# TUMFTM/CamRaDepth

Hardware: AMD Instinct MI355X
Metric: training images/sec at 256x416 bf16 (higher is better)
Workload: dtype bf16; 1 GPU; CamRaDepth base (image+radar) train step, 8x7x256x416 per GPU, bf16 MFMA / fp32 accumulate, diffGradNorm + OneCycleLR, Dropout2d/DropPath on; global_batch=8, parallelism=dp1, hip_graph=True

## Files before the change

camradepth_amd/csrc/decoder_ops.hip:

```cpp
#include "common.h"

namespace {

constexpr int TPB = 256;
__device__ __constant__ float WO[4] = {-0.10546875f, 0.87890625f, 0.26171875f, -0.03515625f};
__device__ __constant__ float WE[4] = {-0.03515625f, 0.26171875f, 0.87890625f, -0.10546875f};

__device__ __forceinline__ void taps_of(int o, int n, int (&idx)[4], float (&w)[4]) {
  const int k = o >> 1;
  const bool odd = o & 1;
  const int base = odd ? k - 1 : k - 2;
#pragma unroll
  for (int t = 0; t < 4; ++t) {
    int i = base + t;
    idx[t] = i < 0 ? 0 : (i > n - 1 ? n - 1 : i);
    w[t] = odd ? WO[t] : WE[t];
  }
}

template <int F8>
__global__ __launch_bounds__(TPB) void k_bicubic(const bf16_t* x, int x_ld, int H, int W, int C, void* y, int y_ld, float inv_scale,
                                                 void* y2, int y2_ld) {
  const int b = blockIdx.y;
  const int CG = C >> 3;
  const int OW = 2 * W;
  const long long total = (long long)H * W * CG;
  const long long i = (long long)blockIdx.x * TPB + threadIdx.x;
  if (i >= total) return;
  const int cg = (int)(i % CG);
  const int pix = (int)(i / CG);
  const int k = pix / W, m = pix - k * W;
  const bf16_t* xb = x + (long long)b * H * W * x_ld + cg * 8;
  int cx[5];
#pragma unroll
  for (int c = 0; c < 5; ++c) { const int ix = m - 2 + c; cx[c] = ix < 0 ? 0 : (ix > W - 1 ? W - 1 : ix); }
  float he[5][8], ho[5][8];
#pragma unroll
  for (int r = 0; r < 5; ++r) {
    int iy = k - 2 + r;
    iy = iy < 0 ? 0 : (iy > H - 1 ? H - 1 : iy);
    float v[5][8];
#pragma unroll
    for (int c = 0; c < 5; ++c) load8(xb, ((long long)iy * W + cx[c]) * x_ld, 0, v[c]);
#pragma unroll
    for (int j = 0; j < 8; ++j) { he[r][j] = 0.f; ho[r][j] = 0.f; }
#pragma unroll
    for (int t = 0; t < 4; ++t)
#pragma unroll
      for (int j = 0; j < 8; ++j) { he[r][j] += WE[t] * v[t][j]; ho[r][j] += WO[t] * v[t + 1][j]; }
  }
#pragma unroll
  for (int oy = 0; oy < 2; ++oy)
#pragma unroll
    for (int ox = 0; ox < 2; ++ox) {
      float out[8];
#pragma unroll
      for (int j = 0; j < 8; ++j) out[j] = 0.f;
#pragma unroll
      for (int t = 0; t < 4; ++t) {
        const float wy = oy ? WO[t] : WE[t];
#pragma unroll
        for (int j = 0; j < 8; ++j) out[j] += wy * (ox ? ho[t + oy][j] : he[t + oy][j]);
      }
      const long long opix = (long long)b * 2 * H * OW + (long long)(2 * k + oy) * OW + 2 * m + ox;
      if (F8) store8_fp8(y, opix * y_ld + cg * 8, out, inv_scale);
      else store8_bf16(y, opix * y_ld + cg * 8, out);
      if (F8 == 2) store8_bf16(y2, opix * y2_ld + cg * 8, out);
    }
}

__device__ __forceinline__ void bwd_weights(int i, int n, float (&w)[10]) {
#pragma unroll
  for (int k = 0; k < 10; ++k) {
    const int o = 2 * i - 4 + k;
    float acc = 0.f;
    if (o >= 0 && o < 2 * n) {
      int idx[4];
      float ww[4];
      taps_of(o, n, idx, ww);
#pragma unroll
      for (int t = 0; t < 4; ++t)
        if (idx[t] == i) acc += ww[t];
    }
    w[k] = acc;
  }
}

__global__ __launch_bounds__(TPB) void k_bicubic_bwd(const bf16_t* dy, int dy_ld, int H, int W, int C, bf16_t* dx, int dx_ld,
                                                     int accumulate) {
  const int b = blockIdx.y;
  const int CG = C >> 3;
  const int OH = 2 * H, OW = 2 * W;
  const long long total = (long long)H * W * CG;
  const long long i = (long long)blockIdx.x * TPB + threadIdx.x;
  if (i >= total) return;
  const int cg = (int)(i % CG);
  const int pix = (int)(i / CG);
  const int iy = pix / W, ix = pix - iy * W;
  float wy[10], wx[10];
  bwd_weights(iy, H, wy);
  bwd_weights(ix, W, wx);
  const bf16_t* db = dy + (long long)b * OH * OW * dy_ld + cg * 8;
  float out[8];
#pragma unroll
  for (int j = 0; j < 8; ++j) out[j] = 0.f;
  const bool border = iy < 2 || iy > H - 3 || ix < 2 || ix > W - 3;
  if (!border) {
#pragma unroll
    for (int a = 1; a < 9; ++a) {
      const int oy = 2 * iy - 4 + a;
#pragma unroll
      for (int c = 1; c < 9; ++c) {
        const int ox = 2 * ix - 4 + c;
        float v[8];
        load8(db, ((long long)oy * OW + ox) * dy_ld, 0, v);
        const float w = wy[a] * wx[c];
#pragma unroll
        for (int j = 0; j < 8; ++j) out[j] += w * v[j];
      }
    }
  } else {
    for (int a = 0; a < 10; ++a) {
      const int oy = 2 * iy - 4 + a;
      if (oy < 0 || oy >= OH || wy[a] == 0.f) continue;
      for (int c = 0; c < 10; ++c) {
        const int ox = 2 * ix - 4 + c;
        if (ox < 0 || ox >= OW || wx[c] == 0.f) continue;
        float v[8];
        load8(db, ((long long)oy * OW + ox) * dy_ld, 0, v);
        const float w = wy[a] * wx[c];
#pragma unroll
        for (int j = 0; j < 8; ++j) out[j] += w * v[j];
      }
    }
  }
  const long long off = ((long long)b * H * W + pix) * dx_ld + cg * 8;
  if (accumulate) {
    float o[8];
    load8(dx, off, 0, o);
#pragma unroll
    for (int j = 0; j < 8; ++j) out[j] += o[j];
  }
  store8_bf16(dx, off, out);
}

__global__ __launch_bounds__(TPB) void k_nchw_to_pm(const float* x, int C, long long HW, bf16_t* y, int y_ld, int Cpad) {
  const int b = blockIdx.y;
  const int CG = Cpad >> 3;
  const long long total = HW * CG;
  for (long long i = (long long)blockIdx.x * TPB + threadIdx.x; i < total; i += (long long)gridDim.x * TPB) {
    const long long p = i % HW;
    const int cg = (int)(i / HW);
    float v[8];
#pragma unroll
    for (int j = 0; j < 8; ++j) {
      const int c = cg * 8 + j;
      v[j] = c < C ? x[((long long)b * C + c) * HW + p] : 0.f;
    }
    store8_bf16(y, ((long long)b * HW + p) * y_ld + cg * 8, v);
  }
}

__global__ __launch_bounds__(TPB) void k_pm_to_nchw(const void* x, int x_f32, int x_ld, int C, long long HW, float* y) {
  const int b = blockIdx.y;
  const long long total = HW * C;
  for (long long i = (long long)blockIdx.x * TPB + threadIdx.x; i < total; i += (long long)gridDim.x * TPB) {
    const long long p = i % HW;
    const int c = (int)(i / HW);
    const long long off = ((long long)b * HW + p) * x_ld + c;
    y[((long long)b * C + c) * HW + p] = x_f32 ? reinterpret_cast<const float*>(x)[off] : bf2f(reinterpret_cast<const bf16_t*>(x)[off]);
  }
}

__global__ __launch_bounds__(TPB) void k_scale_f32(const float* src, float* dst, long long n, float scale) {
  for (long long i = (long long)blockIdx.x * TPB + threadIdx.x; i < n; i += (long long)gridDim.x * TPB) dst[i] = scale * src[i];
}

__global__ __launch_bounds__(TPB) void k_seg_argmax(const float* logits, int ld, long long rows, int C, int num_classes,
                                                    void* y, int y_f32, int y_ld) {
  for (long long r = (long long)blockIdx.x * TPB + threadIdx.x; r < rows; r += (long long)gridDim.x * TPB) {
    const float* p = logits + r * ld;
    float best = p[0];
    int bi = 0;
    for (int c = 1; c < C; ++c) {
      float v = p[c];
      if (v > best) { best = v; bi = c; }
    }
    const float v = (float)bi / (float)num_classes;
    if (y_f32) reinterpret_cast<float*>(y)[r * y_ld] = v;
    else reinterpret_cast<bf16_t*>(y)[r * y_ld] = f2bf(v);
  }
}

__global__ __launch_bounds__(TPB) void k_slice_copy(const bf16_t* src, int s_ld, bf16_t* dst, int d_ld, long long rows, int C,
                                                    int accumulate) {
  const int CG = C >> 3;
  const long long total = rows * CG;
  for (long long i = (long long)blockIdx.x * TPB + threadIdx.x; i < total; i += (long long)gridDim.x * TPB) {
    const int cg = (int)(i % CG);
    const long long r = i / CG;
    uint4 u = *reinterpret_cast<const uint4*>(src + r * s_ld + cg * 8);
    if (accumulate) {
      float a[8], o[8];
      load8(src, r * s_ld + cg * 8, 0, a);
      load8(dst, r * d_ld + cg * 8, 0, o);
#pragma unroll
      for (int j = 0; j < 8; ++j) a[j] += o[j];
      store8_bf16(dst, r * d_ld + cg * 8, a);
    } else {
      *reinterpret_cast<uint4*>(dst + r * d_ld + cg * 8) = u;
    }
  }
}

__global__ __launch_bounds__(TPB) void k_f32_to_bf16_rows(const float* src, int s_ld, bf16_t* dst, int d_ld, long long rows,
                                                          int C, const float* scale, long long rows_per_sample,
                                                          const bf16_t* add, int add_ld, int vec) {
  if (vec) {
    const int CG = C >> 3;
    const long long total = rows * CG;
    for (long long i = (long long)blockIdx.x * TPB + threadIdx.x; i < total; i += (long long)gridDim.x * TPB) {
      const int cg = (int)(i % CG);
      const long long r = i / CG;
      const float s = scale ? scale[r / rows_per_sample] : 1.f;
      float v[8];
      load8(src, r * s_ld + cg * 8, 1, v);
#pragma unroll
      for (int j = 0; j < 8; ++j) v[j] *= s;
      if (add) {
        float a[8];
        load8(add, r * add_ld + cg * 8, 0, a);
#pragma unroll
        for (int j = 0; j < 8; ++j) v[j] += a[j];
      }
      store8_bf16(dst, r * d_ld + cg * 8, v);
    }
    return;
  }
  const long long total = rows * C;
  for (long long i = (long long)blockIdx.x * TPB + threadIdx.x; i < total; i += (long long)gridDim.x * TPB) {
    const int c = (int)(i % C);
    const long long r = i / C;
    float s = scale ? scale[r / rows_per_sample] : 1.f;
    float v = s * src[r * s_ld + c];
    if (add) v += bf2f(add[r * add_ld + c]);
    dst[r * d_ld + c] = f2bf(v);
  }
}

__global__ __launch_bounds__(TPB) void k_sigmoid_bwd(const bf16_t* a, bf16_t* da, long long n8) {
  for (long long i = (long long)blockIdx.x * TPB + threadIdx.x; i < n8; i += (long long)gridDim.x * TPB) {
    float av[8], dv[8];
    load8(a, i * 8, 0, av);
    load8(da, i * 8, 0, dv);
#pragma unroll
    for (int j = 0; j < 8; ++j) dv[j] *= av[j] * (1.f - av[j]);
    store8_bf16(da, i * 8, dv);
  }
}

__global__ __launch_bounds__(TPB) void k_head2_fwd(const bf16_t* a, const float* w, const float* bias, int H, int W,
                                                   float* depth, bf16_t* copy, int copy_ld) {
  const int b = blockIdx.y, q = threadIdx.x & 3;
  float wv[9][8];
#pragma unroll
  for (int t = 0; t < 9; ++t)
#pragma unroll
    for (int j = 0; j < 8; ++j) wv[t][j] = bf_round(w[(q * 8 + j) * 9 + t]);
  const float bias0 = bias[0];
  const bf16_t* ab = a + (long long)b * H * W * 32 + q * 8;
  const int npix = H * W, stride = (gridDim.x * TPB) >> 2;
  for (int pix = (blockIdx.x * TPB + threadIdx.x) >> 2; pix < npix; pix += stride) {
    const int py = pix / W, px = pix - py * W;
    uint4 tv[9];
    bool in[9];
#pragma unroll
    for (int t = 0; t < 9; ++t) {
      const int iy = py + t / 3 - 1, ix = px + t % 3 - 1;
      in[t] = (unsigned)iy < (unsigned)H && (unsigned)ix < (unsigned)W;
      const int cy = iy < 0 ? 0 : (iy < H ? iy : H - 1), cx = ix < 0 ? 0 : (ix < W ? ix : W - 1);
      tv[t] = *reinterpret_cast<const uint4*>(ab + ((long long)cy * W + cx) * 32);
    }
    float acc = 0.f;
#pragma unroll
    for (int t = 0; t < 9; ++t) {
      const uint4 u = in[t] ? tv[t] : make_uint4(0, 0, 0, 0);
      acc += bf_lo(u.x) * wv[t][0]; acc += bf_hi(u.x) * wv[t][1]; acc += bf_lo(u.y) * wv[t][2]; acc += bf_hi(u.y) * wv[t][3];
      acc += bf_lo(u.z) * wv[t][4]; acc += bf_hi(u.z) * wv[t][5]; acc += bf_lo(u.w) * wv[t][6]; acc += bf_hi(u.w) * wv[t][7];
    }
    acc += __shfl_xor(acc, 1);
    acc += __shfl_xor(acc, 2);
    if (q == 0) {
      const float r = bf_round(acc + bias0);
      depth[(long long)b * npix + pix] = r;
      if (copy) copy[((long long)b * npix + pix) * copy_ld] = f2bf(r);
    }
  }
}

__global__ __launch_bounds__(TPB) void k_head2_bwd_data(const float* gd, const bf16_t* add, int add_ld, const bf16_t* a,
                                                        const float* w, int H, int W, bf16_t* dz) {
  const int b = blockIdx.y, q = threadIdx.x & 3;
  float wv[9][8];
#pragma unroll
  for (int t = 0; t < 9; ++t)
#pragma unroll
    for (int j = 0; j < 8; ++j) wv[t][j] = bf_round(w[(q * 8 + j) * 9 + t]);
  const float* gb = gd + (long long)b * H * W;
  const bf16_t* addb = add ? add + (long long)b * H * W * add_ld : nullptr;
  const int npix = H * W, stride = (gridDim.x * TPB) >> 2;
  for (int pix = (blockIdx.x * TPB + threadIdx.x) >> 2; pix < npix; pix += stride) {
    const int py = pix / W, px = pix - py * W;
    float acc[8];
#pragma unroll
    for (int j = 0; j < 8; ++j) acc[j] = 0.f;
    float dyv[9];
    long long oc[9];
    bool in[9];
#pragma unroll
    for (int t = 0; t < 9; ++t) {
      const int oy = py + 1 - t / 3, ox = px + 1 - t % 3;
      in[t] = (unsigned)oy < (unsigned)H && (unsigned)ox < (unsigned)W;
      const int cy = oy < 0 ? 0 : (oy < H ? oy : H - 1), cx = ox < 0 ? 0 : (ox < W ? ox : W - 1);
      oc[t] = (long long)cy * W + cx;
      dyv[t] = gb[oc[t]];
    }
    if (addb) {
      bf16_t av9[9];
#pragma unroll
      for (int t = 0; t < 9; ++t) av9[t] = addb[oc[t] * add_ld];
#pragma unroll
      for (int t = 0; t < 9; ++t) dyv[t] += bf2f(av9[t]);
    }
#pragma unroll
    for (int t = 0; t < 9; ++t) {
      const float dv = in[t] ? bf_round(dyv[t]) : 0.f;
#pragma unroll
      for (int j = 0; j < 8; ++j) acc[j] += dv * wv[t][j];
    }
    float av[8];
    const long long off = ((long long)b * npix + pix) * 32 + q * 8;
    load8(a, off, 0, av);
#pragma unroll
    for (int j = 0; j < 8; ++j) acc[j] *= av[j] * (1.f - av[j]);
    store8_bf16(dz, off, acc);
  }
}

__global__ __launch_bounds__(TPB) void k_head2_wgrad(const float* gd, const bf16_t* add, int add_ld, const bf16_t* a, int H, int W,
                                                     int chunk, crd_sum_t* rows, int replicas) {
  __shared__ float sm[9 * 32 + 1];
  const int b = blockIdx.y, q = threadIdx.x & 3, pl = threadIdx.x >> 2;
  const float* gb = gd + (long long)b * H * W;
  const bf16_t* addb = add ? add + (long long)b * H * W * add_ld : nullptr;
  const bf16_t* ab = a + (long long)b * H * W * 32 + q * 8;
  float acc[9][8], bs = 0.f;
#pragma unroll
  for (int t = 0; t < 9; ++t)
#pragma unroll
    for (int j = 0; j < 8; ++j) acc[t][j] = 0.f;
  int p0 = blockIdx.x * chunk, p1 = p0 + chunk;
  if (p1 > H * W) p1 = H * W;
  for (int pix = p0 + pl; pix < p1; pix += TPB / 4) {
    const int py = pix / W, px = pix - py * W;
    float dyv = gb[pix];
    if (addb) dyv += bf2f(addb[(long long)pix * add_ld]);
    dyv = bf_round(dyv);
    bs += dyv;
    uint4 raw[9];
    float wt[9];
#pragma unroll
    for (int ky = 0; ky < 3; ++ky)
#pragma unroll
      for (int kx = 0; kx < 3; ++kx) {
        const int iy = py + ky - 1, ix = px + kx - 1;
        const int cy = iy < 0 ? 0 : (iy < H ? iy : H - 1), cx = ix < 0 ? 0 : (ix < W ? ix : W - 1);
        raw[ky * 3 + kx] = *reinterpret_cast<const uint4*>(ab + ((long long)cy * W + cx) * 32);
        wt[ky * 3 + kx] = ((unsigned)iy < (unsigned)H && (unsigned)ix < (unsigned)W) ? dyv : 0.f;
      }
#pragma unroll
    for (int t = 0; t < 9; ++t) {
      const uint4 u = raw[t];
      const float v[8] = {bf_lo(u.x), bf_hi(u.x), bf_lo(u.y), bf_hi(u.y), bf_lo(u.z), bf_hi(u.z), bf_lo(u.w), bf_hi(u.w)};
#pragma unroll
      for (int j = 0; j < 8; ++j) acc[t][j] += wt[t] * v[j];
    }
  }
  for (int o = 4; o < 64; o <<= 1) {
#pragma unroll
    for (int t = 0; t < 9; ++t)
#pragma unroll
      for (int j = 0; j < 8; ++j) acc[t][j] += __shfl_xor(acc[t][j], o);
    bs += __shfl_xor(bs, o);
  }
  const int wave = threadIdx.x >> 6, l = threadIdx.x & 63;
  for (int w = 0; w < TPB / 64; ++w) {
    if (wave == w && l < 4) {
#pragma unroll
      for (int t = 0; t < 9; ++t)
#pragma unroll
        for (int j = 0; j < 8; ++j) {
          float* p = &sm[t * 32 + q * 8 + j];
          *p = w == 0 ? acc[t][j] : *p + acc[t][j];
        }
      if (l == 0) sm[288] = w == 0 ? bs : sm[288] + bs;
    }
    __syncthreads();
  }
  crd_sum_t* dst = rows + (long long)((blockIdx.y * gridDim.x + blockIdx.x) % replicas) * 289;
  for (int i = threadIdx.x; i < 288; i += TPB) grad_add(&dst[(i & 31) * 9 + (i >> 5)], sm[i]);
  if (threadIdx.x == 0) grad_add(&dst[288], sm[288]);
}

constexpr int BTH = 8, BTW = 16, BCG = 2;
constexpr int BRH = 2 * BTH + 8, BRW = 2 * BTW + 8;
__global__ __launch_bounds__(TPB) void k_bicubic_bwd_tile(const bf16_t* dy, int dy_ld, int H, int W, int C, bf16_t* dx, int dx_ld,
                                                          int accumulate, int tiles_x) {
  __shared__ __attribute__((aligned(16))) uint4 sdy[BRH * BRW * BCG];
  const int b = blockIdx.z;
  const int g0 = blockIdx.y * BCG;
  const int CG = C >> 3;
  const int tyi = blockIdx.x / tiles_x, txi = blockIdx.x - tyi * tiles_x;
  const int y0 = tyi * BTH, x0 = txi * BTW;
  const int OH = 2 * H, OW = 2 * W;
  const bf16_t* db = dy + (long long)b * OH * OW * dy_ld;
  const int t = threadIdx.x;
  const int g = t & (BCG - 1), xc = (t >> 1) & (BTW - 1), rgp = t >> 5;
  const int ix = x0 + xc, iy = y0 + rgp;
  const bool colok = g0 + g < CG && ix < W;
  float wx[10], wy[10];
  bwd_weights(ix < W ? ix : W - 1, W, wx);
  bwd_weights(iy < H ? iy : H - 1, H, wy);
#pragma unroll
  for (int i = 0; i < 10; ++i) asm volatile("" : "+v"(wx[i]), "+v"(wy[i]));
  {
    constexpr int NP = (BRH * BRW * BCG + TPB - 1) / TPB;
    uint4 r[NP];
#pragma unroll
    for (int k = 0; k < NP; ++k) {
      const int i = t + k * TPB;
      const int px = i / BCG, gg = i - px * BCG;
      const int ry = px / BRW, rx = px - ry * BRW;
      const int oy = 2 * y0 - 4 + ry, ox = 2 * x0 - 4 + rx;
      const bool ok = i < BRH * BRW * BCG && g0 + gg < CG && (unsigned)oy < (unsigned)OH && (unsigned)ox < (unsigned)OW;
      const int cy = oy < 0 ? 0 : (oy < OH ? oy : OH - 1), cx = ox < 0 ? 0 : (ox < OW ? ox : OW - 1), cgr = g0 + gg < CG ? g0 + gg : g0;
      const uint4 u = *reinterpret_cast<const uint4*>(db + ((long long)cy * OW + cx) * dy_ld + cgr * 8);
      r[k] = ok ? u : make_uint4(0, 0, 0, 0);
    }
#pragma unroll
    for (int k = 0; k < NP; ++k) {
      const int i = t + k * TPB;
      if (i < BRH * BRW * BCG) sdy[i] = r[k];
    }
  }
  __syncthreads();
  constexpr int RPT = BRH / 8;
  float hs[RPT][8];
#pragma unroll
  for (int k = 0; k < RPT; ++k) {
    const int ry = k * 8 + rgp;
#pragma unroll
    for (int j = 0; j < 8; ++j) hs[k][j] = 0.f;
#pragma unroll
    for (int c = 0; c < 10; ++c) {
      const uint4 u = sdy[(ry * BRW + 2 * xc + c) * BCG + g];
      const float w = wx[c];
      hs[k][0] += w * bf_lo(u.x); hs[k][1] += w * bf_hi(u.x); hs[k][2] += w * bf_lo(u.y); hs[k][3] += w * bf_hi(u.y);
      hs[k][4] += w * bf_lo(u.z); hs[k][5] += w * bf_hi(u.z); hs[k][6] += w * bf_lo(u.w); hs[k][7] += w * bf_hi(u.w);
    }
  }
  __syncthreads();
  float4* srow = reinterpret_cast<float4*>(sdy);
  constexpr int HALF = BRH * BTW * BCG;
#pragma unroll
  for (int k = 0; k < RPT; ++k) {
    const int ry = k * 8 + rgp;
    float4* p = srow + (ry * BTW + xc) * BCG + g;
    p[0] = make_float4(hs[k][0], hs[k][1], hs[k][2], hs[k][3]);
    p[HALF] = make_float4(hs[k][4], hs[k][5], hs[k][6], hs[k][7]);
  }
  __syncthreads();
  if (!colok || iy >= H) return;
  float out[8];
#pragma unroll
  for (int j = 0; j < 8; ++j) out[j] = 0.f;
#pragma unroll
  for (int a = 0; a < 10; ++a) {
    const float4* p = srow + ((2 * rgp + a) * BTW + xc) * BCG + g;
    const float4 lo = p[0], hi = p[HALF];
    const float w = wy[a];
    out[0] += w * lo.x; out[1] += w * lo.y; out[2] += w * lo.z; out[3] += w * lo.w;
    out[4] += w * hi.x; out[5] += w * hi.y; out[6] += w * hi.z; out[7] += w * hi.w;
  }
  const long long off = ((long long)b * H * W + (long long)iy * W + ix) * dx_ld + (g0 + g) * 8;
  if (accumulate) {
    float o[8];
    load8(dx, off, 0, o);
#pragma unroll
    for (int j = 0; j < 8; ++j) out[j] += o[j];
  }
  store8_bf16(dx, off, out);
}

inline int head2_blocks(int H, int W, int B) {
  long long n = cdiv(4ll * H * W, TPB);
  long long cap = 4096 / (B > 0 ? B : 1);
  if (cap < 1) cap = 1;
  return (int)(n > cap ? cap : n);
}

}

extern "C" int crd_bicubic2x(const void* x, int32_t x_ld, int32_t x_coff, int32_t B, int32_t H, int32_t W, int32_t C, void* y,
                             int32_t y_ld, int32_t y_coff, crd_stream_t stream) {
  CRD_CHECK_ARG(x && y, "crd_bicubic2x: null pointer");
  CRD_CHECK_ARG(C % 8 == 0 && x_ld % 8 == 0 && x_coff % 8 == 0 && y_ld % 8 == 0 && y_coff % 8 == 0, "crd_bicubic2x: alignment");
  const long long total = 4ll * H * W * (C / 8);
  hipLaunchKernelGGL(k_bicubic<0>, dim3((unsigned)cdiv(total / 4, TPB), B), dim3(TPB), 0, as_stream(stream),
                     reinterpret_cast<const bf16_t*>(x) + x_coff, x_ld, H, W, C, reinterpret_cast<bf16_t*>(y) + y_coff, y_ld, 1.f, nullptr, 0);
  CRD_LAUNCH_CHECK("crd_bicubic2x");
  return CRD_OK;
}

extern "C" int crd_bicubic2x_fp8(const void* x, int32_t x_ld, int32_t x_coff, int32_t B, int32_t H, int32_t W, int32_t C, void* y_fp8,
                                 int32_t y_ld, int32_t y_coff, float y_scale, void* y_bf16, int32_t yb_ld, int32_t yb_coff,
                                 crd_stream_t stream) {
  CRD_CHECK_ARG(x && y_fp8 && y_scale > 0.f, "crd_bicubic2x_fp8: null pointer / bad scale");
  CRD_CHECK_ARG(C % 8 == 0 && x_ld % 8 == 0 && x_coff % 8 == 0 && y_ld % 8 == 0 && y_coff % 8 == 0 && yb_ld % 8 == 0 && yb_coff % 8 == 0,
                "crd_bicubic2x_fp8: alignment");
  const long long total = 4ll * H * W * (C / 8);
  const dim3 grid((unsigned)cdiv(total / 4, TPB), B);
  if (y_bf16)
    hipLaunchKernelGGL(k_bicubic<2>, grid, dim3(TPB), 0, as_stream(stream), reinterpret_cast<const bf16_t*>(x) + x_coff, x_ld, H, W, C,
                       reinterpret_cast<unsigned char*>(y_fp8) + y_coff, y_ld, 1.f / y_scale, reinterpret_cast<bf16_t*>(y_bf16) + yb_coff, yb_ld);
  else
    hipLaunchKernelGGL(k_bicubic<1>, grid, dim3(TPB), 0, as_stream(stream), reinterpret_cast<const bf16_t*>(x) + x_coff, x_ld, H, W, C,
                       reinterpret_cast<unsigned char*>(y_fp8) + y_coff, y_ld, 1.f / y_scale, nullptr, 0);
  CRD_LAUNCH_CHECK("crd_bicubic2x_fp8");
  return CRD_OK;
}

extern "C" int crd_bicubic2x_bwd(const void* dy, int32_t dy_ld, int32_t dy_coff, int32_t B, int32_t H, int32_t W, int32_t C,
                                 void* dx, int32_t dx_ld, int32_t dx_coff, int32_t accumulate, crd_stream_t stream) {
  CRD_CHECK_ARG(dy && dx, "crd_bicubic2x_bwd: null pointer");
  CRD_CHECK_ARG(C % 8 == 0 && dy_ld % 8 == 0 && dy_coff % 8 == 0 && dx_ld % 8 == 0 && dx_coff % 8 == 0, "crd_bicubic2x_bwd: alignment");
  if (H >= BTH && W >= BTW) {
    const int tiles_x = cdiv(W, BTW), tiles_y = cdiv(H, BTH);
    hipLaunchKernelGGL(k_bicubic_bwd_tile, dim3(tiles_x * tiles_y, cdiv(C / 8, BCG), B), dim3(TPB), 0, as_stream(stream),
                       reinterpret_cast<const bf16_t*>(dy) + dy_coff, dy_ld, H, W, C, reinterpret_cast<bf16_t*>(dx) + dx_coff, dx_ld,
                       accumulate, tiles_x);
    CRD_LAUNCH_CHECK("crd_bicubic2x_bwd");
    return CRD_OK;
  }
  const long long total = (long long)H * W * (C / 8);
  hipLaunchKernelGGL(k_bicubic_bwd, dim3((unsigned)cdiv(total, TPB), B), dim3(TPB), 0, as_stream(stream),
                     reinterpret_cast<const bf16_t*>(dy) + dy_coff, dy_ld, H, W, C, reinterpret_cast<bf16_t*>(dx) + dx_coff, dx_ld,
                     accumulate);
  CRD_LAUNCH_CHECK("crd_bicubic2x_bwd");
  return CRD_OK;
}

extern "C" int crd_nchw_to_pm(const float* x, int32_t B, int32_t C, int32_t H, int32_t W, void* y, int32_t y_ld, int32_t y_coff,
                              int32_t Cpad, crd_stream_t stream) {
  CRD_CHECK_ARG(x && y, "crd_nchw_to_pm: null pointer");
  CRD_CHECK_ARG(Cpad % 8 == 0 && Cpad >= C && y_ld % 8 == 0 && y_coff % 8 == 0, "crd_nchw_to_pm: alignment");
  const long long HW = (long long)H * W;
  hipLaunchKernelGGL(k_nchw_to_pm, dim3(blocks_for(HW * (Cpad / 8), TPB, 4096), B), dim3(TPB), 0, as_stream(stream), x, C, HW,
                     reinterpret_cast<bf16_t*>(y) + y_coff, y_ld, Cpad);
  CRD_LAUNCH_CHECK("crd_nchw_to_pm");
  return CRD_OK;
}

extern "C" int crd_pm_to_nchw(const void* x, int32_t x_f32, int32_t x_ld, int32_t x_coff, int32_t B, int32_t C, int32_t H,
                              int32_t W, float* y, crd_stream_t stream) {
  CRD_CHECK_ARG(x && y, "crd_pm_to_nchw: null pointer");
  const long long HW = (long long)H * W;
  const void* xp = x_f32 ? (const void*)(reinterpret_cast<const float*>(x) + x_coff) : (const void*)(reinterpret_cast<const bf16_t*>(x) + x_coff);
  hipLaunchKernelGGL(k_pm_to_nchw, dim3(blocks_for(HW * C, TPB, 4096), B), dim3(TPB), 0, as_stream(stream), xp, x_f32, x_ld, C, HW, y);
  CRD_LAUNCH_CHECK("crd_pm_to_nchw");
  return CRD_OK;
}

extern "C" int crd_seg_argmax(const void* logits, int32_t ld, int32_t B, int32_t P, int32_t C, int32_t num_classes, void* y,
                              int32_t y_f32, int32_t y_ld, int32_t y_coff, crd_stream_t stream) {
  CRD_CHECK_ARG(logits && y && C >= 1 && num_classes >= 1, "crd_seg_argmax: bad argument");
  const long long rows = (long long)B * P;
  void* yp = y_f32 ? (void*)(reinterpret_cast<float*>(y) + y_coff) : (void*)(reinterpret_cast<bf16_t*>(y) + y_coff);
  hipLaunchKernelGGL(k_seg_argmax, dim3(blocks_for(rows, TPB, 4096)), dim3(TPB), 0, as_stream(stream), reinterpret_cast<const float*>(logits),
                     ld, rows, C, num_classes, yp, y_f32, y_ld);
  CRD_LAUNCH_CHECK("crd_seg_argmax");
  return CRD_OK;
}

extern "C" int crd_scale_f32(const float* src, float* dst, int64_t n, float scale, crd_stream_t stream) {
  CRD_CHECK_ARG(src && dst && n > 0, "crd_scale_f32: bad argument");
  hipLaunchKernelGGL(k_scale_f32, dim3(blocks_for(n, TPB, 4096)), dim3(TPB), 0, as_stream(stream), src, dst, (long long)n, scale);
  CRD_LAUNCH_CHECK("crd_scale_f32");
  return CRD_OK;
}

extern "C" int crd_slice_copy(const void* src, int32_t s_ld, int32_t s_coff, void* dst, int32_t d_ld, int32_t d_coff,
                              int64_t rows, int32_t C, int32_t accumulate, crd_stream_t stream) {
  CRD_CHECK_ARG(src && dst, "crd_slice_copy: null pointer");
  CRD_CHECK_ARG(C % 8 == 0 && s_ld % 8 == 0 && s_coff % 8 == 0 && d_ld % 8 == 0 && d_coff % 8 == 0, "crd_slice_copy: alignment");
  hipLaunchKernelGGL(k_slice_copy, dim3(blocks_for(rows * (C / 8), TPB, 4096)), dim3(TPB), 0, as_stream(stream),
                     reinterpret_cast<const bf16_t*>(src) + s_coff, s_ld, reinterpret_cast<bf16_t*>(dst) + d_coff, d_ld,
                     (long long)rows, C, accumulate);
  CRD_LAUNCH_CHECK("crd_slice_copy");
  return CRD_OK;
}

extern "C" int crd_f32_to_bf16_rows(const float* src, int32_t s_ld, void* dst, int32_t d_ld, int32_t d_coff, int64_t rows,
                                    int32_t C, const float* scale, int64_t rows_per_sample, const void* add, int32_t add_ld,
                                    int32_t add_coff, crd_stream_t stream) {
  CRD_CHECK_ARG(src && dst && rows_per_sample > 0, "crd_f32_to_bf16_rows: bad argument");
  const int vec = (C % 8 == 0) && (s_ld % 8 == 0) && (d_ld % 8 == 0) && (d_coff % 8 == 0) &&
                  (!add || (add_ld % 8 == 0 && add_coff % 8 == 0)) && ((reinterpret_cast<uintptr_t>(src) & 31) == 0);
  hipLaunchKernelGGL(k_f32_to_bf16_rows, dim3(blocks_for(vec ? rows * (C / 8) : rows * C, TPB, 4096)), dim3(TPB), 0, as_stream(stream), src,
                     s_ld, reinterpret_cast<bf16_t*>(dst) + d_coff, d_ld, (long long)rows, C, scale, (long long)rows_per_sample,
                     add ? reinterpret_cast<const bf16_t*>(add) + add_coff : nullptr, add_ld, vec);
  CRD_LAUNCH_CHECK("crd_f32_to_bf16_rows");
  return CRD_OK;
}

extern "C" int crd_head_conv2_fwd(const void* a, const float* w, const float* bias, int32_t B, int32_t H, int32_t W, float* depth,
                                  void* copy, int32_t copy_ld, int32_t copy_coff, crd_stream_t stream) {
  CRD_CHECK_ARG(a && w && bias && depth, "crd_head_conv2_fwd: null pointer");
  hipLaunchKernelGGL(k_head2_fwd, dim3((unsigned)head2_blocks(H, W, B), B), dim3(TPB), 0, as_stream(stream),
                     reinterpret_cast<const bf16_t*>(a), w, bias, H, W, depth,
                     copy ? reinterpret_cast<bf16_t*>(copy) + copy_coff : nullptr, copy_ld);
  CRD_LAUNCH_CHECK("crd_head_conv2_fwd");
  return CRD_OK;
}

static int head2_bwd_launch(const float* gd, const void* add, int32_t add_ld, int32_t add_coff, const void* a, const float* w,
                            int32_t B, int32_t H, int32_t W, void* dz, crd_sum_t* dw_rows, int32_t replicas, int parts,
                            const char* who, crd_stream_t stream) {
  CRD_CHECK_ARG(gd && a && (!(parts & 1) || (w && dz)) && (!(parts & 2) || (dw_rows && replicas >= 1)), "%s: null pointer / replicas < 1", who);
  const bf16_t* addp = add ? reinterpret_cast<const bf16_t*>(add) + add_coff : nullptr;
  hipStream_t st = as_stream(stream);
  if (parts & 1)
    hipLaunchKernelGGL(k_head2_bwd_data, dim3((unsigned)head2_blocks(H, W, B), B), dim3(TPB), 0, st, gd, addp, add_ld,
                       reinterpret_cast<const bf16_t*>(a), w, H, W, reinterpret_cast<bf16_t*>(dz));
  if (parts & 2) {
    const int P = H * W;
    int nblk = cdiv(P, 64 * 4);
    int cap = 2048 / (B > 0 ? B : 1); if (cap < 1) cap = 1;
    if (nblk > cap) nblk = cap;
    const int chunk = cdiv(P, nblk);
    nblk = cdiv(P, chunk);
    hipLaunchKernelGGL(k_head2_wgrad, dim3(nblk, B), dim3(TPB), 0, st, gd, addp, add_ld, reinterpret_cast<const bf16_t*>(a), H, W, chunk,
                       dw_rows, replicas);
  }
  CRD_LAUNCH_CHECK(who);
  return CRD_OK;
}

extern "C" int crd_head_conv2_bwd(const float* gd, const void* add, int32_t add_ld, int32_t add_coff, const void* a, const float* w,
                                  int32_t B, int32_t H, int32_t W, void* dz, crd_sum_t* dw_rows, int32_t replicas,
                                  crd_stream_t stream) {
  return head2_bwd_launch(gd, add, add_ld, add_coff, a, w, B, H, W, dz, dw_rows, replicas, 3, "crd_head_conv2_bwd", stream);
}

extern "C" int crd_head_conv2_bwd_data(const float* gd, const void* add, int32_t add_ld, int32_t add_coff, const void* a,
                                       const float* w, int32_t B, int32_t H, int32_t W, void* dz, crd_stream_t stream) {
  return head2_bwd_launch(gd, add, add_ld, add_coff, a, w, B, H, W, dz, nullptr, 0, 1, "crd_head_conv2_bwd_data", stream);
}

extern "C" int crd_head_conv2_wgrad(const float* gd, const void* add, int32_t add_ld, int32_t add_coff, const void* a, int32_t B,
                                    int32_t H, int32_t W, crd_sum_t* dw_rows, int32_t replicas, crd_stream_t stream) {
  return head2_bwd_launch(gd, add, add_ld, add_coff, a, nullptr, B, H, W, nullptr, dw_rows, replicas, 2, "crd_head_conv2_wgrad", stream);
}

extern "C" int crd_sigmoid_bwd(const void* a, void* da, int64_t n, crd_stream_t stream) {
  CRD_CHECK_ARG(a && da && n % 8 == 0, "crd_sigmoid_bwd: bad argument");
  hipLaunchKernelGGL(k_sigmoid_bwd, dim3(blocks_for(n / 8, TPB, 4096)), dim3(TPB), 0, as_stream(stream), reinterpret_cast<const bf16_t*>(a),
                     reinterpret_cast<bf16_t*>(da), (long long)(n / 8));
  CRD_LAUNCH_CHECK("crd_sigmoid_bwd");
  return CRD_OK;
}
```

Before: 465.4 images/s.

## Stream vertical strips with rolling row windows in bicubic and head conv kernels

Bicubic upsampling and the 3x3 depth-head forward, backward-data and weight-gradient kernels now give each thread a vertical strip of rows. Each thread keeps a rolling window of horizontally filtered or loaded rows in registers and prefetches the next row, so every input row is read once per strip instead of being reloaded by up to 9 neighbouring output pixels. Head weights are staged through shared memory, and the grid is sized from a target workgroup count with an environment override. The cost is more registers, possible lower occupancy, and fewer threads when strips are long.

```diff
diff --git a/camradepth_amd/csrc/decoder_ops.hip b/camradepth_amd/csrc/decoder_ops.hip
--- a/camradepth_amd/csrc/decoder_ops.hip
+++ b/camradepth_amd/csrc/decoder_ops.hip
@@ -19,54 +19,77 @@
 }
 
 template <int F8>
-__global__ __launch_bounds__(TPB) void k_bicubic(const bf16_t* x, int x_ld, int H, int W, int C, void* y, int y_ld, float inv_scale,
-                                                 void* y2, int y2_ld) {
+__global__ __launch_bounds__(TPB) void k_bicubic(const bf16_t* x, int x_ld, int H, int W, int C, int R, int nstrips, void* y, int y_ld,
+                                                 float inv_scale, void* y2, int y2_ld) {
   const int b = blockIdx.y;
   const int CG = C >> 3;
   const int OW = 2 * W;
-  const long long total = (long long)H * W * CG;
+  const long long total = (long long)nstrips * W * CG;
   const long long i = (long long)blockIdx.x * TPB + threadIdx.x;
   if (i >= total) return;
   const int cg = (int)(i % CG);
-  const int pix = (int)(i / CG);
-  const int k = pix / W, m = pix - k * W;
+  const int col = (int)(i / CG);
+  const int s = col / W, m = col - s * W;
+  const int k0 = s * R, k1 = k0 + R < H ? k0 + R : H;
   const bf16_t* xb = x + (long long)b * H * W * x_ld + cg * 8;
-  int cx[5];
-#pragma unroll
-  for (int c = 0; c < 5; ++c) { const int ix = m - 2 + c; cx[c] = ix < 0 ? 0 : (ix > W - 1 ? W - 1 : ix); }
+  int cxo[5];
+#pragma unroll
+  for (int c = 0; c < 5; ++c) { const int ix = m - 2 + c; cxo[c] = (ix < 0 ? 0 : (ix > W - 1 ? W - 1 : ix)) * x_ld; }
+  auto request = [&](int rel, uint4 (&raw)[5]) {
+    int iy = k0 - 2 + rel;
+    iy = iy < 0 ? 0 : (iy > H - 1 ? H - 1 : iy);
+    const bf16_t* rowp = xb + (long long)iy * W * x_ld;
+#pragma unroll
+    for (int c = 0; c < 5; ++c) raw[c] = *reinterpret_cast<const uint4*>(rowp + cxo[c]);
+  };
+  auto hpass = [&](const uint4 (&raw)[5], float (&e)[8], float (&o)[8]) {
+    float v[5][8];
+#pragma unroll
+    for (int c = 0; c < 5; ++c) unpack8(raw[c], v[c]);
+#pragma unroll
+    for (int j = 0; j < 8; ++j) { e[j] = 0.f; o[j] = 0.f; }
+#pragma unroll
+    for (int t = 0; t < 4; ++t)
+#pragma unroll
+      for (int j = 0; j < 8; ++j) { e[j] += WE[t] * v[t][j]; o[j] += WO[t] * v[t + 1][j]; }
+  };
   float he[5][8], ho[5][8];
-#pragma unroll
-  for (int r = 0; r < 5; ++r) {
-    int iy = k - 2 + r;
-    iy = iy < 0 ? 0 : (iy > H - 1 ? H - 1 : iy);
-    float v[5][8];
-#pragma unroll
-    for (int c = 0; c < 5; ++c) load8(xb, ((long long)iy * W + cx[c]) * x_ld, 0, v[c]);
-#pragma unroll
-    for (int j = 0; j < 8; ++j) { he[r][j] = 0.f; ho[r][j] = 0.f; }
-#pragma unroll
-    for (int t = 0; t < 4; ++t)
-#pragma unroll
-      for (int j = 0; j < 8; ++j) { he[r][j] += WE[t] * v[t][j]; ho[r][j] += WO[t] * v[t + 1][j]; }
-  }
-#pragma unroll
-  for (int oy = 0; oy < 2; ++oy)
-#pragma unroll
-    for (int ox = 0; ox < 2; ++ox) {
-      float out[8];
-#pragma unroll
-      for (int j = 0; j < 8; ++j) out[j] = 0.f;
-#pragma unroll
-      for (int t = 0; t < 4; ++t) {
-        const float wy = oy ? WO[t] : WE[t];
-#pragma unroll
-        for (int j = 0; j < 8; ++j) out[j] += wy * (ox ? ho[t + oy][j] : he[t + oy][j]);
-      }
-      const long long opix = (long long)b * 2 * H * OW + (long long)(2 * k + oy) * OW + 2 * m + ox;
-      if (F8) store8_fp8(y, opix * y_ld + cg * 8, out, inv_scale);
-      else store8_bf16(y, opix * y_ld + cg * 8, out);
-      if (F8 == 2) store8_bf16(y2, opix * y2_ld + cg * 8, out);
-    }
+  uint4 raw[5];
+  {
+    uint4 first[4][5];
+#pragma unroll
+    for (int r = 0; r < 4; ++r) request(r, first[r]);
+    request(4, raw);
+#pragma unroll
+    for (int r = 0; r < 4; ++r) hpass(first[r], he[r], ho[r]);
+  }
+  for (int kb = k0; kb < k1; kb += 5) {
+#pragma unroll
+    for (int u = 0; u < 5; ++u) {
+      const int k = kb + u;
+      if (k >= k1) break;
+      hpass(raw, he[(u + 4) % 5], ho[(u + 4) % 5]);
+      request(k - k0 + 5, raw);
+#pragma unroll
+      for (int oy = 0; oy < 2; ++oy)
+#pragma unroll
+        for (int ox = 0; ox < 2; ++ox) {
+          float out[8];
+#pragma unroll
+          for (int j = 0; j < 8; ++j) out[j] = 0.f;
+#pragma unroll
+          for (int t = 0; t < 4; ++t) {
+            const float wy = oy ? WO[t] : WE[t];
+#pragma unroll
+            for (int j = 0; j < 8; ++j) out[j] += wy * (ox ? ho[(u + t + oy) % 5][j] : he[(u + t + oy) % 5][j]);
+          }
+          const long long opix = (long long)b * 2 * H * OW + (long long)(2 * k + oy) * OW + 2 * m + ox;
+          if (F8) store8_fp8(y, opix * y_ld + cg * 8, out, inv_scale);
+          else store8_bf16(y, opix * y_ld + cg * 8, out);
+          if (F8 == 2) store8_bf16(y2, opix * y2_ld + cg * 8, out);
+        }
+    }
+  }
 }
 
 __device__ __forceinline__ void bwd_weights(int i, int n, float (&w)[10]) {
@@ -259,131 +282,200 @@
   }
 }
 
-__global__ __launch_bounds__(TPB) void k_head2_fwd(const bf16_t* a, const float* w, const float* bias, int H, int W,
-                                                   float* depth, bf16_t* copy, int copy_ld) {
-  const int b = blockIdx.y, q = threadIdx.x & 3;
+constexpr int HEAD2_PL = TPB / 4;
+constexpr int HEAD2_WGS = 3 * 256, HEAD2_WGS_WGRAD = 2 * 256;
+
+__device__ __forceinline__ void head2_weights(const float* w, int q, float (&wv)[9][8]) {
+  __shared__ __attribute__((aligned(16))) float sw[4 * 9 * 8];
+  for (int i = threadIdx.x; i < 288; i += TPB) {
+    const int c = i / 9, t = i - c * 9;
+    sw[(c >> 3) * 72 + t * 8 + (c & 7)] = bf_round(w[i]);
+  }
+  __syncthreads();
+#pragma unroll
+  for (int t = 0; t < 9; ++t)
+#pragma unroll
+    for (int j = 0; j < 8; ++j) wv[t][j] = sw[q * 72 + t * 8 + j];
+}
+
+struct Head2Item { int b, px, y0, y1, cxl, cxr; bool inl, inr; };
+__device__ __forceinline__ Head2Item head2_item(int H, int W, int R, int nstrips, int items) {
+  Head2Item it;
+  const int item = blockIdx.x * HEAD2_PL + (threadIdx.x >> 2);
+  const int col = item < items ? item : 0;
+  const int bs = col / W;
+  it.px = col - bs * W;
+  it.b = bs / nstrips;
+  it.y0 = (bs - it.b * nstrips) * R;
+  it.y1 = item < items ? (it.y0 + R < H ? it.y0 + R : H) : it.y0;
+  it.inl = it.px > 0; it.inr = it.px < W - 1;
+  it.cxl = it.inl ? it.px - 1 : 0; it.cxr = it.inr ? it.px + 1 : W - 1;
+  return it;
+}
+__device__ __forceinline__ void head2_row(const bf16_t* ab, const Head2Item& it, int iy, int H, int W, uint4 (&r)[3], bool& iny) {
+  iny = (unsigned)iy < (unsigned)H;
+  const int cy = iy < 0 ? 0 : (iy < H ? iy : H - 1);
+  const bf16_t* p = ab + (long long)cy * W * 32;
+  r[0] = *reinterpret_cast<const uint4*>(p + it.cxl * 32);
+  r[1] = *reinterpret_cast<const uint4*>(p + it.px * 32);
+  r[2] = *reinterpret_cast<const uint4*>(p + it.cxr * 32);
+}
+
+__global__ __launch_bounds__(TPB) void k_head2_fwd(const bf16_t* a, const float* w, const float* bias, int H, int W, int R, int nstrips,
+                                                   int items, float* depth, bf16_t* copy, int copy_ld) {
+  const int q = threadIdx.x & 3;
   float wv[9][8];
+  head2_weights(w, q, wv);
+  const Head2Item it = head2_item(H, W, R, nstrips, items);
+  if (it.y1 == it.y0) return;
+  const float bias0 = bias[0];
+  const bf16_t* ab = a + (long long)it.b * H * W * 32 + q * 8;
+  const long long obase = (long long)it.b * H * W + it.px;
+  uint4 win[3][3];
+  bool iny[3];
+  head2_row(ab, it, it.y0 - 1, H, W, win[0], iny[0]);
+  head2_row(ab, it, it.y0, H, W, win[1], iny[1]);
+  head2_row(ab, it, it.y0 + 1, H, W, win[2], iny[2]);
+  for (int yb = it.y0; yb < it.y1; yb += 3) {
+#pragma unroll
+    for (int u = 0; u < 3; ++u) {
+      const int py = yb + u;
+      if (py >= it.y1) break;
+      float acc = 0.f;
+#pragma unroll
+      for (int t = 0; t < 9; ++t) {
+        const int sl = (u + t / 3) % 3, kx = t % 3;
+        const bool in = iny[sl] && (kx == 0 ? it.inl : kx == 2 ? it.inr : true);
+        const uint4 v = in ? win[sl][kx] : make_uint4(0, 0, 0, 0);
+        acc += bf_lo(v.x) * wv[t][0]; acc += bf_hi(v.x) * wv[t][1]; acc += bf_lo(v.y) * wv[t][2]; acc += bf_hi(v.y) * wv[t][3];
+        acc += bf_lo(v.z) * wv[t][4]; acc += bf_hi(v.z) * wv[t][5]; acc += bf_lo(v.w) * wv[t][6]; acc += bf_hi(v.w) * wv[t][7];
+        if (t == 2) head2_row(ab, it, py + 2, H, W, win[u], iny[u]);
+      }
+      acc += __shfl_xor(acc, 1);
+      acc += __shfl_xor(acc, 2);
+      if (q == 0) {
+        const float r = bf_round(acc + bias0);
+        const long long o = obase + (long long)py * W;
+        depth[o] = r;
+        if (copy) copy[o * copy_ld] = f2bf(r);
+      }
+    }
+  }
+}
+
+__global__ __launch_bounds__(TPB) void k_head2_bwd_data(const float* gd, const bf16_t* add, int add_ld, const bf16_t* a,
+                                                        const float* w, int H, int W, int R, int nstrips, int items, bf16_t* dz) {
+  const int q = threadIdx.x & 3;
+  float wv[9][8];
+  head2_weights(w, q, wv);
+  const Head2Item it = head2_item(H, W, R, nstrips, items);
+  if (it.y1 == it.y0) return;
+  const float* gb = gd + (long long)it.b * H * W;
+  const bf16_t* addb = add ? add + (long long)it.b * H * W * add_ld : nullptr;
+  const bf16_t* ab = a + (long long)it.b * H * W * 32 + q * 8;
+  bf16_t* dzb = dz + (long long)it.b * H * W * 32 + q * 8;
+  float graw[4][3], dv[4][3];
+  bf16_t araw[4][3];
+  bool iny[4];
+  auto request = [&](int iy, int sl) {
+    iny[sl] = (unsigned)iy < (unsigned)H;
+    const long long o = (long long)(iy < 0 ? 0 : (iy < H ? iy : H - 1)) * W;
+    graw[sl][0] = gb[o + it.cxl]; graw[sl][1] = gb[o + it.px]; graw[sl][2] = gb[o + it.cxr];
+    if (addb) {
+      araw[sl][0] = addb[(o + it.cxl) * add_ld]; araw[sl][1] = addb[(o + it.px) * add_ld]; araw[sl][2] = addb[(o + it.cxr) * add_ld];
+    }
+  };
+  auto settle = [&](int sl) {
+#pragma unroll
+    for (int k = 0; k < 3; ++k) {
+      float v = graw[sl][k];
+      if (addb) v += bf2f(araw[sl][k]);
+      const bool in = iny[sl] && (k == 0 ? it.inl : k == 2 ? it.inr : true);
+      dv[sl][k] = in ? bf_round(v) : 0.f;
+    }
+  };
+  request(it.y0 - 1, 0);
+  request(it.y0, 1);
+  request(it.y0 + 1, 2);
+  uint4 an = *reinterpret_cast<const uint4*>(ab + ((long long)it.y0 * W + it.px) * 32);
+  settle(0);
+  settle(1);
+  for (int yb = it.y0; yb < it.y1; yb += 4) {
+#pragma unroll
+    for (int u = 0; u < 4; ++u) {
+      const int py = yb + u;
+      if (py >= it.y1) break;
+      request(py + 2, (u + 3) & 3);
+      const uint4 ac = an;
+      const long long off = ((long long)py * W + it.px) * 32;
+      an = *reinterpret_cast<const uint4*>(ab + ((long long)(py + 1 < it.y1 ? py + 1 : py) * W + it.px) * 32);
+      settle((u + 2) & 3);
+      float acc[8];
+#pragma unroll
+      for (int j = 0; j < 8; ++j) acc[j] = 0.f;
+#pragma unroll
+      for (int t = 0; t < 9; ++t) {
+        const float d = dv[(u + 2 - t / 3) & 3][2 - t % 3];
+#pragma unroll
+        for (int j = 0; j < 8; ++j) acc[j] += d * wv[t][j];
+      }
+      float av[8];
+      unpack8(ac, av);
+#pragma unroll
+      for (int j = 0; j < 8; ++j) acc[j] *= av[j] * (1.f - av[j]);
+      store8_bf16(dzb, off, acc);
+    }
+  }
+}
+
+__global__ __launch_bounds__(TPB) void k_head2_wgrad(const float* gd, const bf16_t* add, int add_ld, const bf16_t* a, int H, int W,
+                                                     int R, int nstrips, int items, crd_sum_t* rows, int replicas) {
+  __shared__ float sm[9 * 32 + 1];
+  const int q = threadIdx.x & 3;
+  const Head2Item it = head2_item(H, W, R, nstrips, items);
+  const float* gb = gd + (long long)it.b * H * W;
+  const bf16_t* addb = add ? add + (long long)it.b * H * W * add_ld : nullptr;
+  const bf16_t* ab = a + (long long)it.b * H * W * 32 + q * 8;
+  float acc[9][8], bs = 0.f;
 #pragma unroll
   for (int t = 0; t < 9; ++t)
 #pragma unroll
-    for (int j = 0; j < 8; ++j) wv[t][j] = bf_round(w[(q * 8 + j) * 9 + t]);
-  const float bias0 = bias[0];
-  const bf16_t* ab = a + (long long)b * H * W * 32 + q * 8;
-  const int npix = H * W, stride = (gridDim.x * TPB) >> 2;
-  for (int pix = (blockIdx.x * TPB + threadIdx.x) >> 2; pix < npix; pix += stride) {
-    const int py = pix / W, px = pix - py * W;
-    uint4 tv[9];
-    bool in[9];
-#pragma unroll
-    for (int t = 0; t < 9; ++t) {
-      const int iy = py + t / 3 - 1, ix = px + t % 3 - 1;
-      in[t] = (unsigned)iy < (unsigned)H && (unsigned)ix < (unsigned)W;
-      const int cy = iy < 0 ? 0 : (iy < H ? iy : H - 1), cx = ix < 0 ? 0 : (ix < W ? ix : W - 1);
-      tv[t] = *reinterpret_cast<const uint4*>(ab + ((long long)cy * W + cx) * 32);
-    }
-    float acc = 0.f;
-#pragma unroll
-    for (int t = 0; t < 9; ++t) {
-      const uint4 u = in[t] ? tv[t] : make_uint4(0, 0, 0, 0);
-      acc += bf_lo(u.x) * wv[t][0]; acc += bf_hi(u.x) * wv[t][1]; acc += bf_lo(u.y) * wv[t][2]; acc += bf_hi(u.y) * wv[t][3];
-      acc += bf_lo(u.z) * wv[t][4]; acc += bf_hi(u.z) * wv[t][5]; acc += bf_lo(u.w) * wv[t][6]; acc += bf_hi(u.w) * wv[t][7];
-    }
-    acc += __shfl_xor(acc, 1);
-    acc += __shfl_xor(acc, 2);
-    if (q == 0) {
-      const float r = bf_round(acc + bias0);
-      depth[(long long)b * npix + pix] = r;
-      if (copy) copy[((long long)b * npix + pix) * copy_ld] = f2bf(r);
-    }
-  }
-}
-
-__global__ __launch_bounds__(TPB) void k_head2_bwd_data(const float* gd, const bf16_t* add, int add_ld, const bf16_t* a,
-                                                        const float* w, int H, int W, bf16_t* dz) {
-  const int b = blockIdx.y, q = threadIdx.x & 3;
-  float wv[9][8];
-#pragma unroll
-  for (int t = 0; t < 9; ++t)
-#pragma unroll
-    for (int j = 0; j < 8; ++j) wv[t][j] = bf_round(w[(q * 8 + j) * 9 + t]);
-  const float* gb = gd + (long long)b * H * W;
-  const bf16_t* addb = add ? add + (long long)b * H * W * add_ld : nullptr;
-  const int npix = H * W, stride = (gridDim.x * TPB) >> 2;
-  for (int pix = (blockIdx.x * TPB + threadIdx.x) >> 2; pix < npix; pix += stride) {
-    const int py = pix / W, px = pix - py * W;
-    float acc[8];
-#pragma unroll
-    for (int j = 0; j < 8; ++j) acc[j] = 0.f;
-    float dyv[9];
-    long long oc[9];
-    bool in[9];
-#pragma unroll
-    for (int t = 0; t < 9; ++t) {
-      const int oy = py + 1 - t / 3, ox = px + 1 - t % 3;
-      in[t] = (unsigned)oy < (unsigned)H && (unsigned)ox < (unsigned)W;
-      const int cy = oy < 0 ? 0 : (oy < H ? oy : H - 1), cx = ox < 0 ? 0 : (ox < W ? ox : W - 1);
-      oc[t] = (long long)cy * W + cx;
-      dyv[t] = gb[oc[t]];
-    }
-    if (addb) {
-      bf16_t av9[9];
-#pragma unroll
-      for (int t = 0; t < 9; ++t) av9[t] = addb[oc[t] * add_ld];
-#pragma unroll
-      for (int t = 0; t < 9; ++t) dyv[t] += bf2f(av9[t]);
-    }
-#pragma unroll
-    for (int t = 0; t < 9; ++t) {
-      const float dv = in[t] ? bf_round(dyv[t]) : 0.f;
-#pragma unroll
-      for (int j = 0; j < 8; ++j) acc[j] += dv * wv[t][j];
-    }
-    float av[8];
-    const long long off = ((long long)b * npix + pix) * 32 + q * 8;
-    load8(a, off, 0, av);
-#pragma unroll
-    for (int j = 0; j < 8; ++j) acc[j] *= av[j] * (1.f - av[j]);
-    store8_bf16(dz, off, acc);
-  }
-}
-
-__global__ __launch_bounds__(TPB) void k_head2_wgrad(const float* gd, const bf16_t* add, int add_ld, const bf16_t* a, int H, int W,
-                                                     int chunk, crd_sum_t* rows, int replicas) {
-  __shared__ float sm[9 * 32 + 1];
-  const int b = blockIdx.y, q = threadIdx.x & 3, pl = threadIdx.x >> 2;
-  const float* gb = gd + (long long)b * H * W;
-  const bf16_t* addb = add ? add + (long long)b * H * W * add_ld : nullptr;
-  const bf16_t* ab = a + (long long)b * H * W * 32 + q * 8;
-  float acc[9][8], bs = 0.f;
-#pragma unroll
-  for (int t = 0; t < 9; ++t)
-#pragma unroll
     for (int j = 0; j < 8; ++j) acc[t][j] = 0.f;
-  int p0 = blockIdx.x * chunk, p1 = p0 + chunk;
-  if (p1 > H * W) p1 = H * W;
-  for (int pix = p0 + pl; pix < p1; pix += TPB / 4) {
-    const int py = pix / W, px = pix - py * W;
-    float dyv = gb[pix];
-    if (addb) dyv += bf2f(addb[(long long)pix * add_ld]);
-    dyv = bf_round(dyv);
-    bs += dyv;
-    uint4 raw[9];
-    float wt[9];
-#pragma unroll
-    for (int ky = 0; ky < 3; ++ky)
-#pragma unroll
-      for (int kx = 0; kx < 3; ++kx) {
-        const int iy = py + ky - 1, ix = px + kx - 1;
-        const int cy = iy < 0 ? 0 : (iy < H ? iy : H - 1), cx = ix < 0 ? 0 : (ix < W ? ix : W - 1);
-        raw[ky * 3 + kx] = *reinterpret_cast<const uint4*>(ab + ((long long)cy * W + cx) * 32);
-        wt[ky * 3 + kx] = ((unsigned)iy < (unsigned)H && (unsigned)ix < (unsigned)W) ? dyv : 0.f;
+  uint4 win[4][3];
+  bool iny[4];
+  float gn = 0.f;
+  bf16_t adn = 0;
+  auto request_dy = [&](int py) {
+    const long long o = (long long)(py < it.y1 ? py : it.y1 - 1) * W + it.px;
+    gn = gb[o];
+    if (addb) adn = addb[o * add_ld];
+  };
+  if (it.y1 > it.y0) {
+    head2_row(ab, it, it.y0 - 1, H, W, win[0], iny[0]);
+    head2_row(ab, it, it.y0, H, W, win[1], iny[1]);
+    head2_row(ab, it, it.y0 + 1, H, W, win[2], iny[2]);
+    request_dy(it.y0);
+  }
+  for (int yb = it.y0; yb < it.y1; yb += 4) {
+#pragma unroll
+    for (int u = 0; u < 4; ++u) {
+      const int py = yb + u;
+      if (py >= it.y1) break;
+      head2_row(ab, it, py + 2, H, W, win[(u + 3) & 3], iny[(u + 3) & 3]);
+      float dyv = gn;
+      if (addb) dyv += bf2f(adn);
+      request_dy(py + 1);
+      dyv = bf_round(dyv);
+      bs += dyv;
+#pragma unroll
+      for (int t = 0; t < 9; ++t) {
+        const int sl = (u + t / 3) & 3, kx = t % 3;
+        const float wt = (iny[sl] && (kx == 0 ? it.inl : kx == 2 ? it.inr : true)) ? dyv : 0.f;
+        float v[8];
+        unpack8(win[sl][kx], v);
+#pragma unroll
+        for (int j = 0; j < 8; ++j) acc[t][j] += wt * v[j];
       }
-#pragma unroll
-    for (int t = 0; t < 9; ++t) {
-      const uint4 u = raw[t];
-      const float v[8] = {bf_lo(u.x), bf_hi(u.x), bf_lo(u.y), bf_hi(u.y), bf_lo(u.z), bf_hi(u.z), bf_lo(u.w), bf_hi(u.w)};
-#pragma unroll
-      for (int j = 0; j < 8; ++j) acc[t][j] += wt[t] * v[j];
     }
   }
   for (int o = 4; o < 64; o <<= 1) {
@@ -502,11 +594,31 @@
   store8_bf16(dx, off, out);
 }
 
-inline int head2_blocks(int H, int W, int B) {
-  long long n = cdiv(4ll * H * W, TPB);
-  long long cap = 4096 / (B > 0 ? B : 1);
-  if (cap < 1) cap = 1;
-  return (int)(n > cap ? cap : n);
+constexpr int HEAD2_MIN_ROWS = 4;
+struct Head2Runs { int R, nstrips, items; unsigned blocks; };
+inline Head2Runs head2_runs(int B, int H, int W, int wgs) {
+  Head2Runs g;
+  const long long lanes = (long long)crd_dev_int("CRD_HEAD2_WGS", wgs) * HEAD2_PL;
+  long long R = ((long long)B * H * W + lanes - 1) / lanes;
+  const int rmin = crd_dev_int("CRD_HEAD2_MIN_ROWS", HEAD2_MIN_ROWS);
+  if (R < rmin) R = rmin;
+  if (R > H) R = H;
+  g.nstrips = cdiv(H, R);
+  g.R = cdiv(H, g.nstrips);
+  g.items = B * g.nstrips * W;
+  g.blocks = (unsigned)cdiv(g.items, HEAD2_PL);
+  return g;
+}
+
+constexpr int BICUBIC_ROWS = 8;
+struct BicubicRuns { int R, nstrips; unsigned blocks; };
+inline BicubicRuns bicubic_runs(int B, int H, int W, int C) {
+  BicubicRuns g;
+  g.R = crd_dev_int("CRD_BICUBIC_ROWS", BICUBIC_ROWS);
+  while (g.R > 1 && (long long)B * cdiv(H, g.R) * W * (C / 8) < 256 * 4 * 64) g.R >>= 1;
+  g.nstrips = cdiv(H, g.R);
+  g.blocks = (unsigned)cdiv((long long)g.nstrips * W * (C / 8), TPB);
+  return g;
 }
 
 }
@@ -515,9 +627,9 @@
                              int32_t y_ld, int32_t y_coff, crd_stream_t stream) {
   CRD_CHECK_ARG(x && y, "crd_bicubic2x: null pointer");
   CRD_CHECK_ARG(C % 8 == 0 && x_ld % 8 == 0 && x_coff % 8 == 0 && y_ld % 8 == 0 && y_coff % 8 == 0, "crd_bicubic2x: alignment");
-  const long long total = 4ll * H * W * (C / 8);
-  hipLaunchKernelGGL(k_bicubic<0>, dim3((unsigned)cdiv(total / 4, TPB), B), dim3(TPB), 0, as_stream(stream),
-                     reinterpret_cast<const bf16_t*>(x) + x_coff, x_ld, H, W, C, reinterpret_cast<bf16_t*>(y) + y_coff, y_ld, 1.f, nullptr, 0);
+  const BicubicRuns g = bicubic_runs(B, H, W, C);
+  hipLaunchKernelGGL(k_bicubic<0>, dim3(g.blocks, B), dim3(TPB), 0, as_stream(stream), reinterpret_cast<const bf16_t*>(x) + x_coff, x_ld,
+                     H, W, C, g.R, g.nstrips, reinterpret_cast<bf16_t*>(y) + y_coff, y_ld, 1.f, nullptr, 0);
   CRD_LAUNCH_CHECK("crd_bicubic2x");
   return CRD_OK;
 }
@@ -528,14 +640,15 @@
   CRD_CHECK_ARG(x && y_fp8 && y_scale > 0.f, "crd_bicubic2x_fp8: null pointer / bad scale");
   CRD_CHECK_ARG(C % 8 == 0 && x_ld % 8 == 0 && x_coff % 8 == 0 && y_ld % 8 == 0 && y_coff % 8 == 0 && yb_ld % 8 == 0 && yb_coff % 8 == 0,
                 "crd_bicubic2x_fp8: alignment");
-  const long long total = 4ll * H * W * (C / 8);
-  const dim3 grid((unsigned)cdiv(total / 4, TPB), B);
+  const BicubicRuns g = bicubic_runs(B, H, W, C);
+  const dim3 grid(g.blocks, B);
   if (y_bf16)
     hipLaunchKernelGGL(k_bicubic<2>, grid, dim3(TPB), 0, as_stream(stream), reinterpret_cast<const bf16_t*>(x) + x_coff, x_ld, H, W, C,
-                       reinterpret_cast<unsigned char*>(y_fp8) + y_coff, y_ld, 1.f / y_scale, reinterpret_cast<bf16_t*>(y_bf16) + yb_coff, yb_ld);
+                       g.R, g.nstrips, reinterpret_cast<unsigned char*>(y_fp8) + y_coff, y_ld, 1.f / y_scale,
+                       reinterpret_cast<bf16_t*>(y_bf16) + yb_coff, yb_ld);
   else
     hipLaunchKernelGGL(k_bicubic<1>, grid, dim3(TPB), 0, as_stream(stream), reinterpret_cast<const bf16_t*>(x) + x_coff, x_ld, H, W, C,
-                       reinterpret_cast<unsigned char*>(y_fp8) + y_coff, y_ld, 1.f / y_scale, nullptr, 0);
+                       g.R, g.nstrips, reinterpret_cast<unsigned char*>(y_fp8) + y_coff, y_ld, 1.f / y_scale, nullptr, 0);
   CRD_LAUNCH_CHECK("crd_bicubic2x_fp8");
   return CRD_OK;
 }
@@ -626,9 +739,10 @@
 extern "C" int crd_head_conv2_fwd(const void* a, const float* w, const float* bias, int32_t B, int32_t H, int32_t W, float* depth,
                                   void* copy, int32_t copy_ld, int32_t copy_coff, crd_stream_t stream) {
   CRD_CHECK_ARG(a && w && bias && depth, "crd_head_conv2_fwd: null pointer");
-  hipLaunchKernelGGL(k_head2_fwd, dim3((unsigned)head2_blocks(H, W, B), B), dim3(TPB), 0, as_stream(stream),
-                     reinterpret_cast<const bf16_t*>(a), w, bias, H, W, depth,
-                     copy ? reinterpret_cast<bf16_t*>(copy) + copy_coff : nullptr, copy_ld);
+  CRD_CHECK_ARG(B >= 1 && H >= 1 && W >= 1 && (long long)B * H * W < (1ll << 31), "crd_head_conv2_fwd: bad shape");
+  const Head2Runs g = head2_runs(B, H, W, HEAD2_WGS);
+  hipLaunchKernelGGL(k_head2_fwd, dim3(g.blocks), dim3(TPB), 0, as_stream(stream), reinterpret_cast<const bf16_t*>(a), w, bias, H, W,
+                     g.R, g.nstrips, g.items, depth, copy ? reinterpret_cast<bf16_t*>(copy) + copy_coff : nullptr, copy_ld);
   CRD_LAUNCH_CHECK("crd_head_conv2_fwd");
   return CRD_OK;
 }
@@ -639,19 +753,14 @@
   CRD_CHECK_ARG(gd && a && (!(parts & 1) || (w && dz)) && (!(parts & 2) || (dw_rows && replicas >= 1)), "%s: null pointer / replicas < 1", who);
   const bf16_t* addp = add ? reinterpret_cast<const bf16_t*>(add) + add_coff : nullptr;
   hipStream_t st = as_stream(stream);
+  CRD_CHECK_ARG(B >= 1 && H >= 1 && W >= 1 && (long long)B * H * W < (1ll << 31), "%s: bad shape", who);
+  const Head2Runs g = head2_runs(B, H, W, HEAD2_WGS), gw = head2_runs(B, H, W, HEAD2_WGS_WGRAD);
   if (parts & 1)
-    hipLaunchKernelGGL(k_head2_bwd_data, dim3((unsigned)head2_blocks(H, W, B), B), dim3(TPB), 0, st, gd, addp, add_ld,
-                       reinterpret_cast<const bf16_t*>(a), w, H, W, reinterpret_cast<bf16_t*>(dz));
-  if (parts & 2) {
-    const int P = H * W;
-    int nblk = cdiv(P, 64 * 4);
-    int cap = 2048 / (B > 0 ? B : 1); if (cap < 1) cap = 1;
-    if (nblk > cap) nblk = cap;
-    const int chunk = cdiv(P, nblk);
-    nblk = cdiv(P, chunk);
-    hipLaunchKernelGGL(k_head2_wgrad, dim3(nblk, B), dim3(TPB), 0, st, gd, addp, add_ld, reinterpret_cast<const bf16_t*>(a), H, W, chunk,
-                       dw_rows, replicas);
-  }
+    hipLaunchKernelGGL(k_head2_bwd_data, dim3(g.blocks), dim3(TPB), 0, st, gd, addp, add_ld, reinterpret_cast<const bf16_t*>(a), w, H, W,
+                       g.R, g.nstrips, g.items, reinterpret_cast<bf16_t*>(dz));
+  if (parts & 2)
+    hipLaunchKernelGGL(k_head2_wgrad, dim3(gw.blocks), dim3(TPB), 0, st, gd, addp, add_ld, reinterpret_cast<const bf16_t*>(a), H, W,
+                       gw.R, gw.nstrips, gw.items, dw_rows, replicas);
   CRD_LAUNCH_CHECK(who);
   return CRD_OK;
 }
```

After: 465.3 images/s, median of 2. No clear change (-0.0%).
